# gabry1998/Self-Supervised-Anomaly-Detection

Measured on AMD Instinct MI355X. Metric: train images/sec + anomaly-maps/sec, ResNet-18 256x256 bs256, higher is better.
Workload: dtype f32; 1 GPU; ResNet-18 256x256 bs256 self-sup train + anomaly map, 1xMI355X, synthetic images (BASELINE configs[1]); images_per_gpu=256, global_batch=256, patches_per_image=841, bank_rows=588, parallelism=dp1 (256 images), train_step_launch=hipGraph segments, train_graph_segments=1

## Files before the change

### include/ssad.h

```cpp
#ifndef SSAD_H
#define SSAD_H
#include <stddef.h>
#include <stdint.h>

#ifdef __cplusplus
extern "C" {
#endif

#define SSAD_VERSION 100

int ssad_version(void);
const char* ssad_last_error(void);

int ssad_repack_oihw_to_ohwi(const float* w_oihw, float* w_ohwi, int O, int I, int KH, int KW, void* stream);
int ssad_repack_ohwi_to_oihw(const float* w_ohwi, float* w_oihw, int O, int I, int KH, int KW, void* stream);
int ssad_pack_stem_weight(const float* w_oihw, float* wk, void* stream);
int ssad_pack_stem_weight_ohwi(const float* w_ohwi, float* wk, void* stream);

int ssad_stem_fwd(const float* img, int B, int H, int W, int patch_dim, int patch_stride, int Hv, int Wv,
                  const float* wk, const float* scale, const float* shift, int relu, int hwnc, float* out, void* stream);
int ssad_stem_stats_rows(void);
int ssad_stem_fwd_stats(const float* img, int B, int H, int W, int Hv, int Wv, const float* wk, float* out, float eps,
                        float momentum, float* mean, float* invstd, float* running_mean, float* running_var, double* workspace,
                        void* stream);
// ... 11 lines not shown
int ssad_conv_igemm_fwd(const float* in, const float* w_ohwi, float* out, const float* scale, const float* shift,
                        const float* residual, int relu, int64_t N, int H, int W, int Cin, int Cout, int KH, int KW,
                        int stride, int pad, void* stream);

int ssad_conv_igemm_fwd_hwnc(const float* in, const float* w_ohwi, float* out, const float* scale, const float* shift,
                             const float* residual, int relu, int64_t N, int H, int W, int Cin, int Cout, int KH, int KW,
                             int stride, int pad, void* stream);

int ssad_conv_igemm_fwd_hwnc_ring(const float* in, const float* w_ohwi, float* out, const float* scale, const float* shift,
                                  const float* residual, int relu, int64_t N, int H, int W, int Cin, int Cout, int KH, int KW,
                                  int stride, int pad, int skip_lo, int skip_hi, void* stream);
int ssad_patch_gather_hwnc(const float* dense, float* out, int64_t B, int prow, int pcol, int shift, int Hd, int Wd, int C,
                           int H, int W, int lo, int hi, void* stream);
int ssad_patch_gather_hwnc_band(const float* dense, float* out, int64_t B, int prow, int pcol, int shift, int Hd, int Wd, int C,
                                int H, int W, int lo, int hi, int ilo, int ihi, void* stream);

int ssad_conv_igemm_tile(int64_t N, int H, int W, int Cin, int Cout, int KH, int KW, int stride, int pad, int mode);
int ssad_conv_igemm_tile_id(int64_t N, int H, int W, int Cin, int Cout, int KH, int KW, int stride, int pad, int mode);

int ssad_gap_fwd(const float* in, float* out, int64_t N, int HW, int C, int out_stride, int out_offset, int hwnc,
                 void* stream);

int ssad_l2_normalize_rows(const float* x, float* out, int64_t N, int D, void* stream);
int ssad_cosine_knn_mean(const float* sim, float* out, int64_t Nq, int Nb, int k, void* stream);

int ssad_blur_relu_bilinear(const float* maps, float* out, int n, int h, int w, int ksize, int target, void* stream);

int ssad_gradcam_map(const float* act, const float* alpha, float* out, int64_t B, int HW, int C, int alpha_stride,
                     void* stream);

// ... 292 lines not shown
```

### self-supervised-anomaly-detection_amd/csrc/conv_igemm.hip

```cpp
#include "common.h"
#include <stdlib.h>
#include <type_traits>

#ifndef IGEMM_ABL
#define IGEMM_ABL 0
#endif
#ifndef IGEMM_VAR
#define IGEMM_VAR 4
#endif
#ifndef IGEMM_EPI
#define IGEMM_EPI 1
#endif


#ifndef IGEMM_BUFLD
#define IGEMM_BUFLD 1
#endif

#ifndef IGEMM_TRACE
#define IGEMM_TRACE 0
#endif
#if IGEMM_TRACE
__device__ unsigned long long* g_ig_trace;
#define IG_STAMP(i) do { if (threadIdx.x == 0 && g_ig_trace) g_ig_trace[((size_t)blockIdx.y * gridDim.x + blockIdx.x) * 8 + (i)] = __builtin_readcyclecounter(); } while (0)
// ... 15 lines not shown
    const float* shift;
    const float* residual;
    const uint8_t* res_mask;
    int64_t M;
    int64_t N;
    int H, W, Cin, Ho, Wo, Cout, KH, KW, stride, pad, relu;
    int K;
    int hwnc;
    int cls_start[5];
    int cls_id[4];
    double* stats;
    int skip_lo, skip_hi;
    int pos_lpt;
    int pos_sg;
    int pos_chunk;
    unsigned char pos_tab[64];
};

template <int BM, int BN, int TM, int TN, int BK, int TS, bool POS, bool DB = true, int BF = 0, bool IO = false>
__global__ __launch_bounds__((BM / (32 * TM)) * (BN / (32 * TN)) * 64, (TM * TN > 8 || (TM * TN == 8 && BK >= 32)) ? 1 : 2)
void conv_igemm_f32_kernel(ConvParams p) {
    static_assert(!IO || BF == 2, "half tensors go with fp16 operands");
    using io_t = std::conditional_t<IO, hf, float>;
    constexpr int PE = IO ? 8 : 4;
    constexpr int NT = (BM / (32 * TM)) * (BN / (32 * TN)) * 64;
    constexpr int LDK = BF == 6 ? 3 * BK + 8 : (BF == 3 ? 2 * BK + 8 : (BF ? BK + 8 : BK + 4));
    constexpr int ESZ = BF ? 2 : 4;
    constexpr int CPR = BK / PE;
    constexpr int RPP = NT / CPR;
    constexpr int WN = BN / (32 * TN);
    constexpr int AR = BM / RPP;
// ... 4 lines not shown
    extern __shared__ __attribute__((aligned(16))) float lds[];

    const int tid = threadIdx.x, lane = tid & 63, wave = tid >> 6;
    const int r = lane & 31, h = lane >> 5;
    const int wm = wave / WN, wn = wave % WN;
    const int n0 = blockIdx.y * BN;
    IG_STAMP(0);
#if IGEMM_TRACE
    if (threadIdx.x == 0 && g_ig_trace)
        g_ig_trace[((size_t)blockIdx.y * gridDim.x + blockIdx.x) * 8 + 7] =
            ((unsigned long long)__builtin_amdgcn_s_getreg((31 << 11) | 20) << 32) | __builtin_amdgcn_s_getreg((31 << 11) | 4);
#endif
    const int sc = tid % CPR, sr = tid / CPR;
    const int HoWo = p.Ho * p.Wo;
    const int ntaps = p.KH * p.KW;
    const int64_t in_sp = p.hwnc ? p.N * p.Cin : (int64_t)p.Cin;
    const int64_t in_sn = p.hwnc ? (int64_t)p.Cin : (int64_t)p.H * p.W * p.Cin;
    const io_t* zero = (const io_t*)g_zero_page;
    const io_t* const tin = (const io_t*)p.in;
    const io_t* const twt = (const io_t*)p.wt;

    int64_t m0;
    int pos = 0;
    unsigned tapmask = ntaps >= 32 ? ~0u : ((1u << ntaps) - 1);
    if (POS) {
        if (p.pos_lpt == 2) {
            const unsigned x = blockIdx.x & 7, j = blockIdx.x >> 3;
            const unsigned per_blk = (unsigned)p.pos_chunk * (unsigned)HoWo;
            const unsigned blk = j / per_blk, r = j - blk * per_blk;
            const unsigned pi = r / (unsigned)p.pos_chunk, g = r - pi * (unsigned)p.pos_chunk;
            const unsigned sg = (blk * (unsigned)p.pos_chunk + g) * 8u + x;
            if (sg >= (unsigned)p.pos_sg) return;
            pos = p.pos_tab[pi];
            m0 = (int64_t)sg * BM;
        } else if (p.pos_lpt) {
            const unsigned per_chunk = (unsigned)p.pos_chunk * (unsigned)HoWo;
            const unsigned chunk = blockIdx.x / per_chunk, in_chunk = blockIdx.x - chunk * per_chunk;
            const unsigned first = chunk * (unsigned)p.pos_chunk;
            const unsigned here = min((unsigned)p.pos_chunk, (unsigned)p.pos_sg - first);
            const unsigned pi = in_chunk / here;
            if (pi >= (unsigned)HoWo) return;
            pos = p.pos_tab[pi];
            m0 = (int64_t)(first + in_chunk - pi * here) * BM;
        } else {
        const int stream = blockIdx.x & 31;
        const int64_t j = blockIdx.x >> 5;
        const int64_t q = j / HoWo;
        pos = (int)(j - q * HoWo);
        m0 = (q * 32 + stream) * BM;
        }
        if (m0 >= p.N) return;
        const int oy = pos / p.Wo, ox = pos - oy * p.Wo;
        if (oy >= p.skip_lo && oy <= p.skip_hi && ox >= p.skip_lo && ox <= p.skip_hi) return;
        tapmask = 0;
        for (int ky = 0, t = 0; ky < p.KH; ++ky)
            for (int kx = 0; kx < p.KW; ++kx, ++t) {
                const int y = oy * p.stride - p.pad + ky, x = ox * p.stride - p.pad + kx;
                if ((unsigned)y < (unsigned)p.H && (unsigned)x < (unsigned)p.W) tapmask |= 1u << t;
            }
    } else {
        m0 = (int64_t)blockIdx.x * BM;
    }
    int cpy = 0, cpx = 0, Hc = 1, Wc = 1;
// ... 24 lines not shown
            return ok;
        }
        const bool ok = m < p.M;
        const int64_t mm = ok ? m : 0;
        n = mm / HoWo;
        const int rem = (int)(mm - n * HoWo);
        oy = rem / p.Wo;
        ox = rem - oy * p.Wo;
        return ok;
    };

    constexpr bool BUFA = IGEMM_BUFLD != 0, BUFB = IGEMM_BUFLD != 0;
    constexpr unsigned OOB = 0x80000000u;
    constexpr int SRD3 = 0x00020000;
    int64_t a_org = 0;
    unsigned a_voff[AR], b_voff[BR];
    const io_t* a_ptr[AR];
    unsigned a_mask[AR];
    int a_iy[AR], a_ix[AR];
#pragma unroll
    for (int i = 0; i < AR; ++i) {
        const int64_t m = m0 + sr + RPP * i;
        int64_t n;
        int oy, ox;
        bool ok;
        if (POS) {
            ok = m < p.N;
            n = ok ? m : 0;
            oy = pos / p.Wo;
            ox = pos - oy * p.Wo;
        } else {
            ok = decode_row(m, n, oy, ox);
        }
        const int iy0 = oy * p.stride - p.pad, ix0 = ox * p.stride - p.pad;
        a_iy[i] = iy0;
        a_ix[i] = ix0;
        unsigned mk = 0;
        if (POS) {
            mk = ok ? tapmask : 0u;
        } else if (ok) {
            for (int ky = 0, t = 0; ky < p.KH; ++ky)
                for (int kx = 0; kx < p.KW; ++kx, ++t) {
                    int y = iy0 + ky, x = ix0 + kx;
                    bool v = true;
                    if (TS > 1) {
                        v = y >= 0 && x >= 0 && (y % TS) == 0 && (x % TS) == 0;
                        y /= TS;
                        x /= TS;
                    }
                    if (v && (unsigned)y < (unsigned)p.H && (unsigned)x < (unsigned)p.W) mk |= 1u << t;
                }
            mk &= tapmask;
        }
        a_mask[i] = (IGEMM_ABL & 2) ? 0u : mk;
        a_ptr[i] = TS > 1 ? tin + n * in_sn + sc * PE : tin + n * in_sn + ((int64_t)iy0 * p.W + ix0) * in_sp + sc * PE;
        if (BUFA) {
            if (POS) {
                a_org = m0 * in_sn + ((int64_t)iy0 * p.W + ix0) * in_sp;
                a_voff[i] = (ok && !(IGEMM_ABL & 2)) ? (unsigned)(((int64_t)(sr + RPP * i) * in_sn + sc * PE) * (int64_t)sizeof(io_t)) : OOB;
            } else if (TS > 1) {
                const int64_t nf = (m0 < Mc ? m0 : 0) / (Hc * Wc);
                const int mg = (p.pad + 1) / 2;
                a_org = nf * in_sn - ((int64_t)mg * p.W + mg) * in_sp;
                const int64_t R = (n - nf) * in_sn + ((int64_t)((oy - cpy) / 2 + mg) * p.W + (ox - cpx) / 2 + mg) * in_sp + sc * PE;
                a_voff[i] = ok ? (unsigned)(R * (int64_t)sizeof(io_t)) : OOB;
            } else {
                const int64_t nf = (m0 < p.M ? m0 : 0) / HoWo;
                a_org = nf * in_sn - ((int64_t)p.pad * p.W + p.pad) * in_sp;
                const int64_t R = (n - nf) * in_sn + ((int64_t)(iy0 + p.pad) * p.W + ix0 + p.pad) * in_sp + sc * PE;
                a_voff[i] = ok ? (unsigned)(R * (int64_t)sizeof(io_t)) : OOB;
            }
        }
    }
    const io_t* b_ptr[BR];
// ... 380 lines not shown
    {
        float sum = 0.f;
#pragma unroll
        for (int i = 0; i < TM; ++i)
#pragma unroll
            for (int j = 0; j < TN; ++j)
#pragma unroll
                for (int e = 0; e < 16; ++e) sum += acc[i][j][e];
        if (sum == 123.456f) p.out[0] = sum;
        return;
    }
#endif
    {
    int64_t R0 = m0, RS = 1, limit = p.M - m0;
    if (POS) {
        limit = p.N - m0;
        if (p.hwnc) { R0 = (int64_t)pos * p.N + m0; RS = 1; }
        else { R0 = m0 * HoWo + pos; RS = HoWo; }
    }
    if (IGEMM_EPI && !IO && TS == 1 && limit >= BM && n0 + BN <= p.Cout) {
        const int64_t pitch = RS * p.Cout;
        const int lrow0 = wm * 32 * TM + 4 * h;
        const int colb = n0 + wn * 32 * TN + r;
        const int64_t lane_off = (R0 + (int64_t)lrow0 * RS) * p.Cout + colb;
        float* outp = p.out + lane_off;
        float scl[TN], sft[TN];
#pragma unroll
        for (int j = 0; j < TN; ++j) {
            scl[j] = p.scale ? p.scale[colb + 32 * j] : 1.f;
            sft[j] = p.shift ? p.shift[colb + 32 * j] : 0.f;
        }
        double st0[TN], st1[TN];
// ... 141 lines not shown
                st0 += v;
                st1 += v * v;
            }
        }
        int64_t o[NPASS];
        f32x4 res[NPASS];
        f16x4 rraw[NPASS];
        unsigned mkq[NPASS];
#pragma unroll
        for (int q = 0; q < NPASS; ++q) {
            const int lr = rr + q * RP;
            int64_t row = m0 + ((lr >> 5) * TM + i) * 32 + (lr & 31);
            bool ok = col_ok;
            if (POS) {
                ok = ok && row < p.N;
                row = p.hwnc ? (int64_t)pos * p.N + row : row * HoWo + pos;
            } else if (TS > 1) {
                int64_t n;
                int oy, ox;
                ok = decode_row(row, n, oy, ox) && ok;
                row = (n * p.Ho + oy) * p.Wo + ox;
            } else {
                ok = ok && row < p.M;
            }
            o[q] = ok ? row * p.Cout + col : -1;
            if (IO) rraw[q] = *(const f16x4*)((aligned && ok && p.residual) ? (const void*)((const hf*)p.residual + o[q]) : (const void*)g_zero_page);
            else res[q] = *(const f32x4*)((aligned && ok && p.residual) ? p.residual + o[q] : g_zero_page);
            mkq[q] = 0xfu;
            if (aligned && ok && p.res_mask) mkq[q] = p.res_mask[o[q] >> 2];
        }
#pragma unroll
// ... 79 lines not shown
    constexpr int stage_bytes = (DB ? 2 : 1) * (BM + BN) *
                                (BF == 6 ? (3 * BK + 8) * 2 : (BF == 3 ? (2 * BK + 8) * 2 : (BF ? (BK + 8) * 2 : (BK + 4) * 4)));
    constexpr int epi_bytes = (BM / TM) * (BN + 4) * 4;
    constexpr int lds_min = (stage_bytes > epi_bytes ? stage_bytes : epi_bytes) + ((IGEMM_ABL & 64) ? 40 * 1024 : 0);
    static const int lds_pad = getenv(BN == 64 ? "SSAD_CONV_LDS_PAD_64" : "SSAD_CONV_LDS_PAD_128")
                                   ? atoi(getenv(BN == 64 ? "SSAD_CONV_LDS_PAD_64" : "SSAD_CONV_LDS_PAD_128")) : 0;
    const int lds_bytes = lds_min + lds_pad;
    static bool attr_set = false;
    if (!attr_set) {
        (void)hipFuncSetAttribute((const void*)conv_igemm_f32_kernel<BM, BN, TM, TN, BK, TS, POS, DB, BF, IO>,
                                  hipFuncAttributeMaxDynamicSharedMemorySize, lds_bytes);
        attr_set = true;
    }
    ConvParams q = p;
    q.pos_lpt = 0;
    if (POS) sort_positions(q, (int)cdiv64(p.N, BM));
    int64_t gx = POS ? (q.pos_lpt == 2 ? cdiv64(cdiv64(q.pos_sg, 8), q.pos_chunk) * q.pos_chunk * p.Ho * p.Wo * 8
                        : q.pos_lpt ? cdiv64(q.pos_sg, q.pos_chunk) * q.pos_chunk * p.Ho * p.Wo
                                    : cdiv64(cdiv64(p.N, BM), 32) * 32 * p.Ho * p.Wo)
                     : cdiv64(p.M, BM);
    if (TS > 1) {
        int taps[4];
        for (int c = 0; c < 4; ++c) {
            taps[c] = 0;
            for (int ky = 0; ky < p.KH; ++ky)
                for (int kx = 0; kx < p.KW; ++kx)
                    taps[c] += (((c >> 1) - p.pad + ky) & 1) == 0 && (((c & 1) - p.pad + kx) & 1) == 0;
            q.cls_id[c] = c;
        }
        for (int i = 1; i < 4; ++i)
            for (int j = i; j > 0 && taps[q.cls_id[j]] > taps[q.cls_id[j - 1]]; --j) { int t = q.cls_id[j]; q.cls_id[j] = q.cls_id[j - 1]; q.cls_id[j - 1] = t; }
        gx = 0;
        for (int c = 0; c < 4; ++c) {
            q.cls_start[c] = (int)gx;
// ... 87 lines not shown
        default: return launch<128, 128, 2, 2, 32, TS, POS>(p, st);
    }
}

enum IgemmEntry { E_FWD = 0, E_HWNC = 1, E_RING = 2, E_STATS = 3, E_DGRAD = 4 };

static bool posmajor_rows(IgemmEntry e, const ConvParams& p) {
    if (e == E_HWNC || e == E_RING) return true;
    return e == E_FWD && p.pad > 0 && p.N >= 128 && p.Ho * p.Wo <= 4;
}

static ConvParams dgrad_params(int64_t N, int Hy, int Wy, int Cout, int Hx, int Wx, int Cin, int KH, int KW, int pad) {
    ConvParams p;
    p.pos_lpt = 0; p.pos_sg = 0; p.pos_chunk = 1;
    p.skip_lo = 1; p.skip_hi = 0;
    p.in = nullptr; p.wt = nullptr; p.out = nullptr; p.scale = nullptr; p.shift = nullptr; p.residual = nullptr; p.res_mask = nullptr;
    p.H = Hy; p.W = Wy; p.Cin = Cout; p.Cout = Cin; p.KH = KH; p.KW = KW; p.relu = 0;
    p.stride = 1; p.pad = KH - 1 - pad; p.N = N; p.hwnc = 0;
    p.Ho = Hx; p.Wo = Wx; p.stats = nullptr;
    p.M = N * Hx * Wx;
    p.K = KH * KW * Cout;
    return p;
}

static bool tile_span_ok(const ConvParams& p, bool posmajor, int elt_bytes, int ts = 1) {
    const int64_t image = (int64_t)p.H * p.W * p.Cin * elt_bytes;
    if (posmajor) return p.hwnc || 256 * image < ((int64_t)1 << 31);
    const int64_t rows_per_image = ts > 1 ? (int64_t)(p.Ho / 2) * (p.Wo / 2) : (int64_t)p.Ho * p.Wo;
    return (256 / (rows_per_image > 0 ? rows_per_image : 1) + 2) * image < ((int64_t)1 << 31);
}

int conv_fwd_impl(const float* in, const float* w_ohwi, float* out, const float* scale, const float* shift,
                  const float* residual, int relu, int64_t N, int H, int W, int Cin, int Cout, int KH, int KW, int stride,
                  int pad, int hwnc, void* stream, int bf16 = 0, double* stats = nullptr, int* stat_rows = nullptr, int io16 = 0,
                  int skip_lo = 1, int skip_hi = 0) {
    SSAD_CHECK_ARG(in && w_ohwi && out, "null pointer");
    SSAD_CHECK_ARG(!io16 || (bf16 == 2 && !hwnc && Cout % 4 == 0), "half tensors: fp16 operands, NHWC, Cout % 4 == 0");
    SSAD_CHECK_ARG(N > 0 && H > 0 && W > 0 && Cin > 0 && Cout > 0, "empty shape");
    if ((bf16 == 0 || bf16 == 1 || bf16 == 2) && !io16 && !hwnc && KH == 1 && KW == 1 && H == 1 && W == 1 && stride == 1 && pad == 0 &&
        ssad_linear_small_ok(in, w_ohwi, N, Cin))
        return ssad_linear_small_launch(in, w_ohwi, out, scale, shift, residual, relu, (int)N, Cin, Cout, stats, stat_rows, stream, bf16);
    SSAD_CHECK_ARG(Cin % KALIGN == 0, "Cin must be a multiple of 32");
    SSAD_CHECK_ARG(KH > 0 && KW > 0 && stride > 0 && pad >= 0 && KH * KW <= 32, "bad filter geometry (<= 32 taps)");
    ConvParams p;
    p.pos_lpt = 0; p.pos_sg = 0; p.pos_chunk = 1;
    p.skip_lo = skip_lo; p.skip_hi = skip_hi;
    SSAD_CHECK_ARG(skip_lo > skip_hi || hwnc, "a skipped rectangle of output positions: position-major tensors only");
    p.in = in; p.wt = w_ohwi; p.out = out; p.scale = scale; p.shift = shift; p.residual = residual; p.res_mask = nullptr;
    p.H = H; p.W = W; p.Cin = Cin; p.Cout = Cout; p.KH = KH; p.KW = KW; p.stride = stride; p.pad = pad; p.relu = relu;
    p.Ho = (H + 2 * pad - KH) / stride + 1;
    p.Wo = (W + 2 * pad - KW) / stride + 1;
    SSAD_CHECK_ARG(p.Ho > 0 && p.Wo > 0, "empty output");
    p.M = N * p.Ho * p.Wo;
    p.N = N;
    p.K = KH * KW * Cin;
    p.hwnc = hwnc;
    p.stats = stats;
    const bool posmajor = posmajor_rows(hwnc ? (skip_lo <= skip_hi ? E_RING : E_HWNC) : stats ? E_STATS : E_FWD, p);
    SSAD_CHECK_ARG(cdiv64(p.M, 128) + 32 * p.Ho * p.Wo < (int64_t)2147483647, "M too large for one launch");
    SSAD_CHECK_ARG(tile_span_ok(p, posmajor, io16 ? 2 : 4), "input images too large: the rows of a tile must span less than 2 GB");
    hipStream_t st = (hipStream_t)stream;
    int rows;
    SSAD_CHECK_ARG(bf16 == 0 || bf16 == 1 || bf16 == 2 || bf16 == 3 || bf16 == 6,
                   "operand mode: 0 (fp32), 1 (bf16), 2 (fp16), 3 (bf16x3), 6 (bf16x6)");
    if (bf16 == 6) {
        rows = posmajor ? dispatch_x6<1, true>(p, st) : dispatch_x6<1, false>(p, st);
    } else if (bf16 == 3) {
        rows = posmajor ? dispatch_x3<1, true>(p, st) : dispatch_x3<1, false>(p, st);
    } else if (bf16) {
// ... 59 lines not shown
extern "C" int ssad_conv_igemm_fwd_hwnc(const float* in, const float* w_ohwi, float* out, const float* scale,
                                        const float* shift, const float* residual, int relu, int64_t N, int H, int W,
                                        int Cin, int Cout, int KH, int KW, int stride, int pad, void* stream) {
    return conv_fwd_impl(in, w_ohwi, out, scale, shift, residual, relu, N, H, W, Cin, Cout, KH, KW, stride, pad, 1, stream);
}

extern "C" int ssad_conv_igemm_fwd_hwnc_ring(const float* in, const float* w_ohwi, float* out, const float* scale,
                                             const float* shift, const float* residual, int relu, int64_t N, int H, int W,
                                             int Cin, int Cout, int KH, int KW, int stride, int pad, int skip_lo, int skip_hi,
                                             void* stream) {
    SSAD_CHECK_ARG(skip_lo >= 0 && skip_hi < H && skip_hi < W, "skipped square outside the map");
    return conv_fwd_impl(in, w_ohwi, out, scale, shift, residual, relu, N, H, W, Cin, Cout, KH, KW, stride, pad, 1, stream, 0, nullptr,
                         nullptr, 0, skip_lo, skip_hi);
}

extern "C" int ssad_conv_igemm_tile_id(int64_t N, int H, int W, int Cin, int Cout, int KH, int KW, int stride, int pad, int mode) {
    const int Ho = (H + 2 * pad - KH) / stride + 1, Wo = (W + 2 * pad - KW) / stride + 1;
    ConvParams p;
    if (mode == E_DGRAD) {
        p = dgrad_params(N, Ho, Wo, Cout, H, W, Cin, KH, KW, pad);
    } else {
        p.N = N; p.H = H; p.W = W; p.Cin = Cin; p.Cout = Cout; p.KH = KH; p.KW = KW; p.stride = stride; p.pad = pad;
        p.skip_lo = mode == E_RING ? 0 : 1; p.skip_hi = 0;
        p.Ho = Ho; p.Wo = Wo;
        p.M = N * p.Ho * p.Wo;
    }
    if (posmajor_rows((IgemmEntry)mode, p)) return 100 + (int)pick_tile<true>(p);
    const IgemmTile t = pick_tile<false>(p);
    return t == T_256x256 ? T_128x128 : (int)t;
}

extern "C" int ssad_conv_igemm_tile(int64_t N, int H, int W, int Cin, int Cout, int KH, int KW, int stride, int pad, int mode) {
    static const int dims[13][3] = {{256, 64, 16}, {256, 64, 32}, {128, 64, 32}, {256, 128, 32}, {256, 128, 32}, {128, 256, 32},
                                    {64, 64, 32}, {128, 128, 32}, {256, 256, 32}, {128, 64, 32}, {128, 64, 16}, {128, 128, 16}, {128, 256, 16}};
    const int id = ssad_conv_igemm_tile_id(N, H, W, Cin, Cout, KH, KW, stride, pad, mode), t = id % 100;
    const int code = dims[t][0] * 100000 + dims[t][1] * 100 + dims[t][2];
    return id >= 100 ? -code : code;
}
// ... 103 lines not shown
```

### self-supervised-anomaly-detection_amd/csrc/misc.hip

```cpp
#include "common.h"
#include <stdarg.h>

static thread_local char g_err[512] = "";

void ssad_set_error(const char* fmt, ...) {
    va_list ap;
    va_start(ap, fmt);
    vsnprintf(g_err, sizeof(g_err), fmt, ap);
    va_end(ap);
}

extern "C" const char* ssad_last_error(void) { return g_err; }
extern "C" int ssad_version(void) { return 100; }

namespace {

__global__ void repack_kernel(const float* __restrict__ src, float* __restrict__ dst, int O, int I, int KH, int KW,
                              int to_ohwi) {
    int64_t idx = (int64_t)blockIdx.x * blockDim.x + threadIdx.x;
    int64_t total = (int64_t)O * I * KH * KW;
    if (idx >= total) return;
    int ci = (int)(idx % I);
    int64_t t = idx / I;
    int kx = (int)(t % KW); t /= KW;
// ... 305 lines not shown
    const int64_t N = B * prow * pcol;
    const int side = hi - lo + 1;
    const int iside = ilo > ihi ? 0 : ihi - ilo + 1;
    SSAD_CHECK_ARG(cdiv64(N * (C / 4), 256) < (int64_t)2147483647 && side * side <= 65535, "too large for one launch");
    hipLaunchKernelGGL(patch_gather_hwnc_kernel, dim3((unsigned)cdiv64(N * (C / 4), 256), side * side - iside * iside), dim3(256), 0,
                       (hipStream_t)stream, (const f32x4*)dense, (f32x4*)out, N, prow, pcol, shift, Hd, Wd, C / 4, W, lo, side, ilo, iside);
    SSAD_CHECK_LAUNCH();
    return 0;
}

extern "C" int ssad_patch_gather_hwnc(const float* dense, float* out, int64_t B, int prow, int pcol, int shift, int Hd, int Wd, int C,
                                      int H, int W, int lo, int hi, void* stream) {
    return ssad_patch_gather_hwnc_band(dense, out, B, prow, pcol, shift, Hd, Wd, C, H, W, lo, hi, 1, 0, stream);
}

extern "C" int ssad_gradcam_map(const float* act, const float* alpha, float* out, int64_t B, int HW, int C, int alpha_stride,
                                void* stream) {
    SSAD_CHECK_ARG(act && alpha && out && B > 0 && HW > 0 && C > 0 && alpha_stride >= C, "bad argument");
    const int64_t rows = B * HW;
    hipLaunchKernelGGL(gradcam_map_kernel, dim3((unsigned)cdiv64(rows, 4)), dim3(256), 0, (hipStream_t)stream, act, alpha, out,
                       rows, HW, C, alpha_stride);
    SSAD_CHECK_LAUNCH();
    return 0;
}

extern "C" int ssad_l2_normalize_rows(const float* x, float* out, int64_t N, int D, void* stream) {
    SSAD_CHECK_ARG(x && out && N > 0 && D > 0, "bad argument");
    hipLaunchKernelGGL(l2norm_rows_kernel, dim3((unsigned)cdiv64(N, 4)), dim3(256), 0, (hipStream_t)stream, x, out, N, D);
    SSAD_CHECK_LAUNCH();
    return 0;
// ... 33 lines not shown
```

### self-supervised-anomaly-detection_amd/self_supervised/_hip.py

```python
import ctypes
import os

import torch

_HERE = os.path.dirname(os.path.abspath(__file__))
LIB_PATH = os.path.join(os.path.dirname(_HERE), "lib", "libssad_hip.so")

_c_fp = ctypes.c_void_p
_c_i = ctypes.c_int
_c_l = ctypes.c_int64
_c_f = ctypes.c_float

SIGNATURES = {
    "ssad_repack_oihw_to_ohwi": [_c_fp, _c_fp, _c_i, _c_i, _c_i, _c_i, _c_fp],
    "ssad_repack_ohwi_to_oihw": [_c_fp, _c_fp, _c_i, _c_i, _c_i, _c_i, _c_fp],
    "ssad_pack_stem_weight": [_c_fp, _c_fp, _c_fp],
    "ssad_pack_stem_weight_ohwi": [_c_fp, _c_fp, _c_fp],
    "ssad_pack_stem_weight16_ohwi": [_c_fp, _c_fp, _c_i, _c_fp],
    "ssad_stem_fwd": [_c_fp, _c_i, _c_i, _c_i, _c_i, _c_i, _c_i, _c_i, _c_fp, _c_fp, _c_fp, _c_i, _c_i, _c_fp, _c_fp],
    "ssad_stem_stats_rows": [],
    "ssad_stem_fwd_stats": [_c_fp, _c_i, _c_i, _c_i, _c_i, _c_i, _c_fp, _c_fp, _c_f, _c_f, _c_fp, _c_fp, _c_fp, _c_fp, _c_fp, _c_fp],
    "ssad_pack_stem_weight_folded": [_c_fp, _c_fp, _c_fp],
    "ssad_stem_patch_pool_fwd": [_c_fp, _c_i, _c_i, _c_i, _c_i, _c_fp, _c_fp, _c_fp, _c_i, _c_fp, _c_fp],
    "ssad_stem_patch_pool_fwd_ring": [_c_fp, _c_i, _c_i, _c_i, _c_i, _c_fp, _c_fp, _c_fp, _c_i, _c_i, _c_i, _c_fp, _c_fp],
    "ssad_stem_patch_border_fwd": [_c_fp, _c_i, _c_i, _c_i, _c_i, _c_fp, _c_fp, _c_fp, _c_fp, _c_fp],
    "ssad_maxpool3x3s2_fwd": [_c_fp, _c_fp, _c_l, _c_i, _c_i, _c_i, _c_i, _c_fp],
    "ssad_conv_igemm_fwd": [_c_fp, _c_fp, _c_fp, _c_fp, _c_fp, _c_fp, _c_i, _c_l, _c_i, _c_i, _c_i, _c_i, _c_i, _c_i,
                            _c_i, _c_i, _c_fp],
    "ssad_conv_igemm_fwd_hwnc": [_c_fp, _c_fp, _c_fp, _c_fp, _c_fp, _c_fp, _c_i, _c_l, _c_i, _c_i, _c_i, _c_i, _c_i, _c_i,
                                 _c_i, _c_i, _c_fp],
    "ssad_conv_igemm_fwd_hwnc_ring": [_c_fp, _c_fp, _c_fp, _c_fp, _c_fp, _c_fp, _c_i, _c_l, _c_i, _c_i, _c_i, _c_i, _c_i, _c_i,
                                      _c_i, _c_i, _c_i, _c_i, _c_fp],
    "ssad_patch_gather_hwnc": [_c_fp, _c_fp, _c_l, _c_i, _c_i, _c_i, _c_i, _c_i, _c_i, _c_i, _c_i, _c_i, _c_i, _c_fp],
    "ssad_patch_gather_hwnc_band": [_c_fp, _c_fp, _c_l, _c_i, _c_i, _c_i, _c_i, _c_i, _c_i, _c_i, _c_i, _c_i, _c_i, _c_i, _c_i, _c_fp],
    "ssad_conv_igemm_tile": [_c_l, _c_i, _c_i, _c_i, _c_i, _c_i, _c_i, _c_i, _c_i, _c_i],
    "ssad_conv_igemm_tile_id": [_c_l, _c_i, _c_i, _c_i, _c_i, _c_i, _c_i, _c_i, _c_i, _c_i],
    "ssad_gap_fwd": [_c_fp, _c_fp, _c_l, _c_i, _c_i, _c_i, _c_i, _c_i, _c_fp],
    "ssad_l2_normalize_rows": [_c_fp, _c_fp, _c_l, _c_i, _c_fp],
    "ssad_cosine_knn_mean": [_c_fp, _c_fp, _c_l, _c_i, _c_i, _c_fp],
    "ssad_cosine_knn_fused": [_c_fp, _c_fp, _c_fp, _c_l, _c_i, _c_i, _c_i, _c_fp],
    "ssad_cosine_knn_split": [_c_fp, _c_fp, _c_fp, _c_fp, _c_l, _c_i, _c_i, _c_i, _c_i, _c_fp],
    "ssad_coreset_greedy": [_c_fp, _c_l, _c_i, _c_i, _c_l, _c_i, _c_fp, _c_fp, _c_fp, _c_fp, _c_fp, _c_fp],
    "ssad_gaussian_fit_stats": [_c_fp, _c_l, _c_i, _c_i, _c_fp, _c_fp, _c_fp, _c_fp],
    "ssad_mahalanobis_fused": [_c_fp, _c_fp, _c_fp, _c_fp, _c_fp, _c_l, _c_i, _c_i, _c_fp],
    "ssad_blur_relu_bilinear": [_c_fp, _c_fp, _c_i, _c_i, _c_i, _c_i, _c_i, _c_fp],
    "ssad_flip_transpose_weight": [_c_fp, _c_fp, _c_i, _c_i, _c_i, _c_i, _c_fp],
    "ssad_flip_transpose_batch": [_c_fp, _c_fp, ctypes.POINTER(ctypes.c_int64), _c_i, _c_fp],
    "ssad_conv_igemm_dgrad": [_c_fp, _c_fp, _c_fp, _c_fp, _c_l, _c_i, _c_i, _c_i, _c_i, _c_i, _c_i, _c_i, _c_i, _c_i, _c_i,
                              _c_fp],
# ... 206 lines not shown
```

### self-supervised-anomaly-detection_amd/self_supervised/engine.py

```python
import torch
from torch import nn

import os as _os

from . import ops

BLOCKS = [("layer1", 64, 64, 1), ("layer2", 64, 128, 2), ("layer3", 128, 256, 2), ("layer4", 256, 512, 2)]


def math_mode():
    m = _os.environ.get("SSAD_MATH", "f32").lower()
    return 6 if m in ("bf16x6", "x6") else 3 if m in ("bf16x3", "x3") else 0


class _Block(nn.Module):

    def __init__(self, cin, cout, stride):
        super().__init__()
        self.conv1 = nn.Conv2d(cin, cout, 3, stride, 1, bias=False)
        self.bn1 = nn.BatchNorm2d(cout)
        self.conv2 = nn.Conv2d(cout, cout, 3, 1, 1, bias=False)
        self.bn2 = nn.BatchNorm2d(cout)
        self.downsample = None
        if stride != 1 or cin != cout:
# ... 116 lines not shown
    return pooled


def _trunk_eval_dedup(plan, x, patch_stride, layer_outputs, pooled, conv):
    b, _, h, w = x.shape
    prow, pcol = (h - 32) // patch_stride + 1, (w - 32) // patch_stride + 1
    shift = patch_stride // 2
    band = _os.environ.get("SSAD_GATHER_BAND", "1") != "0"
    dn = ops.stem_fwd(x, plan.stem_w, plan.stem_s, plan.stem_t, True, resize_to=(2 * h, 2 * w))
    dn = ops.maxpool3x3s2_fwd(dn)
    if band and _os.environ.get("SSAD_STEM_BORDER", "1") != "0":
        a = ops.stem_patch_border_fwd(x, plan.stem_wf, plan.stem_s, plan.stem_t, patch_stride)
        ops.patch_gather_hwnc(dn, a, prow, pcol, shift, 2, 14, 4, 12)
    else:
        a = ops.stem_patch_pool_fwd(x, plan.stem_wf, plan.stem_s, plan.stem_t, patch_stride, True, (4, 12) if band else None)
    offs, off = {}, 0
    for k in ("layer1", "layer2", "layer3"):
        if k in layer_outputs:
            offs[k] = off
            off += {"layer1": 64, "layer2": 128, "layer3": 256}[k]
    offs["layer4"] = off
    for i, (name, d) in enumerate(plan.blocks):
        s = d["stride"]
        if name == "layer1":
            lo, hi = 3 + 2 * i, 13 - 2 * i
            dt = ops.conv3x3_c64_eval(dn, d["w1"], d["s1"], d["t1"], None, True)
            dn2 = ops.conv3x3_c64_eval(dt, d["w2"], d["s2"], d["t2"], dn, True)
            t = ops.conv_fwd_hwnc_ring(a, d["w1"], d["s1"], d["t1"], None, True, lo, hi)
            ops.patch_gather_hwnc(dt, t, prow, pcol, shift, lo, hi, *((lo + 2, hi - 2) if band else (1, 0)))
            a2 = ops.conv_fwd_hwnc_ring(t, d["w2"], d["s2"], d["t2"], a, True, lo + 1, hi - 1)
            ops.patch_gather_hwnc(dn2, a2, prow, pcol, shift, lo + 1, hi - 1, *((lo + 3, hi - 3) if band and i == 0 else (1, 0)))
            a, dn = a2, dn2
        else:
            idt = a
            if "wd" in d:
                idt = conv(a, d["wd"], d["sd"], d["td"], None, False, s, 0)
            t = conv(a, d["w1"], d["s1"], d["t1"], None, True, s, 1)
            a = conv(t, d["w2"], d["s2"], d["t2"], idt, True, 1, 1)
        if i % 2 == 1 and name in offs:
            ops.gap_fwd(a, pooled, offs[name], True)
    return pooled


def head_eval(plan, pooled):
    f = pooled
# ... 6 lines not shown
```

### self-supervised-anomaly-detection_amd/self_supervised/ops.py

```python
import os

import torch

from . import _hip


PROFILE = None


def _new(shape, like):
    return torch.empty(shape, device=like.device, dtype=torch.float32)


def _newh(shape, like):
    return torch.empty(shape, device=like.device, dtype=torch.float16)


def _is_h(t):
    return t is not None and t.dtype == torch.float16


def _p(t, allow_none=False):
    return _hip.ptr(t, allow_none, torch.float16 if _is_h(t) else torch.float32)

# ... 257 lines not shown

def conv_fwd_hwnc_ring(x, w_ohwi, scale, shift, residual, relu, skip_lo, skip_hi):
    h, w, n, cin = x.shape
    cout, kh, kw, cin2 = w_ohwi.shape
    assert cin == cin2 and (kh, kw) == (3, 3) and 0 <= skip_lo <= skip_hi < min(h, w)
    out = _new((h, w, n, cout), x)
    side = skip_hi - skip_lo + 1
    ring = h * w - side * side
    taps = _inbounds_taps(h, w, 3, 3, 1, 1) - 9 * side * side if PROFILE is not None else 0
    _run("conv_igemm_pos_f32", 2.0 * n * ring * cout * 9 * cin, 4.0 * (x.numel() + n * ring * cout * (2 if residual is not None else 1) + w_ohwi.numel()),
         lambda: _hip.lib().ssad_conv_igemm_fwd_hwnc_ring(_hip.ptr(x), _hip.ptr(w_ohwi), _hip.ptr(out), _hip.ptr(scale, True),
                                                          _hip.ptr(shift, True), _hip.ptr(residual, True), int(relu), n, h, w,
                                                          cin, cout, 3, 3, 1, 1, skip_lo, skip_hi, _hip.stream()),
         exec_flops=2.0 * n * cout * cin * taps if PROFILE is not None else None,
         tile=lambda: igemm_tile_name(n, h, w, cin, cout, 3, 3, 1, 1, IGEMM_RING))
    return out


def patch_gather_hwnc(dense, out, prow, pcol, shift, lo, hi, ilo=1, ihi=0):
    b, hd, wd, c = dense.shape
    h, w, n, c2 = out.shape
    assert c == c2 and n == b * prow * pcol
    side, iside = hi - lo + 1, max(ihi - ilo + 1, 0)
    _run("patch_gather", 0.0, 8.0 * n * (side * side - iside * iside) * c,
         lambda: _hip.lib().ssad_patch_gather_hwnc_band(_hip.ptr(dense), _hip.ptr(out), b, prow, pcol, shift, hd, wd, c, h, w, lo, hi,
                                                        ilo, ihi, _hip.stream()))
    return out


def conv_fwd(x, w_ohwi, scale=None, shift=None, residual=None, relu=False, stride=1, pad=0, bf16=False):
# ... 895 lines not shown
```

Measured before the change: 8191 images/sec.

## Share overlapping ring-strip conv outputs between neighbouring patches instead of recomputing

In the patch-wise anomaly-map path, overlapping patches (stride smaller than the computed window) recompute identical ring conv outputs. The ring conv is split into strip launches that compute only the non-overlapping windows and edge rows of patches, using a listed position table and a row remapping. A new copy kernel then fills the shared strip positions from neighbouring patches. This cuts redundant FLOPs in layer1 ring convs, at the cost of more launches, extra copy traffic and complex index maps.

```diff
diff --git a/include/ssad.h b/include/ssad.h
--- a/include/ssad.h
+++ b/include/ssad.h
@@ -49,6 +49,13 @@
                            int H, int W, int lo, int hi, void* stream);
 int ssad_patch_gather_hwnc_band(const float* dense, float* out, int64_t B, int prow, int pcol, int shift, int Hd, int Wd, int C,
                                 int H, int W, int lo, int hi, int ilo, int ihi, void* stream);
+
+int ssad_conv_igemm_fwd_hwnc_strip(const float* in, const float* w_ohwi, float* out, const float* scale, const float* shift,
+                                   const float* residual, int relu, int64_t N, int H, int W, int Cin, int Cout, int KH, int KW,
+                                   int stride, int pad, int skip_lo, int skip_hi, int corners, int tb_lo, int tb_hi, int lr_lo,
+                                   int lr_hi, int row_P, int row_S, int row_O, int64_t rows, void* stream);
+int ssad_patch_strip_copy_hwnc(float* out, int64_t B, int prow, int pcol, int shift, int C, int H, int W, int lo, int hi,
+                               void* stream);
 
 int ssad_conv_igemm_tile(int64_t N, int H, int W, int Cin, int Cout, int KH, int KW, int stride, int pad, int mode);
 int ssad_conv_igemm_tile_id(int64_t N, int H, int W, int Cin, int Cout, int KH, int KW, int stride, int pad, int mode);
diff --git a/self-supervised-anomaly-detection_amd/csrc/conv_igemm.hip b/self-supervised-anomaly-detection_amd/csrc/conv_igemm.hip
--- a/self-supervised-anomaly-detection_amd/csrc/conv_igemm.hip
+++ b/self-supervised-anomaly-detection_amd/csrc/conv_igemm.hip
@@ -53,7 +53,10 @@
     int pos_lpt;
     int pos_sg;
     int pos_chunk;
-    unsigned char pos_tab[64];
+    int pos_cnt;
+    int row_P, row_S, row_O;
+    int64_t Nt;
+    unsigned char pos_tab[256];
 };
 
 template <int BM, int BN, int TM, int TN, int BK, int TS, bool POS, bool DB = true, int BF = 0, bool IO = false>
@@ -88,7 +91,7 @@
     const int sc = tid % CPR, sr = tid / CPR;
     const int HoWo = p.Ho * p.Wo;
     const int ntaps = p.KH * p.KW;
-    const int64_t in_sp = p.hwnc ? p.N * p.Cin : (int64_t)p.Cin;
+    const int64_t in_sp = p.hwnc ? p.Nt * p.Cin : (int64_t)p.Cin;
     const int64_t in_sn = p.hwnc ? (int64_t)p.Cin : (int64_t)p.H * p.W * p.Cin;
     const io_t* zero = (const io_t*)g_zero_page;
     const io_t* const tin = (const io_t*)p.in;
@@ -119,8 +122,10 @@
         } else {
         const int stream = blockIdx.x & 31;
         const int64_t j = blockIdx.x >> 5;
-        const int64_t q = j / HoWo;
-        pos = (int)(j - q * HoWo);
+        const int npos = p.pos_cnt ? p.pos_cnt : HoWo;
+        const int64_t q = j / npos;
+        pos = (int)(j - q * npos);
+        if (p.pos_cnt) pos = p.pos_tab[pos];
         m0 = (q * 32 + stream) * BM;
         }
         if (m0 >= p.N) return;
@@ -175,6 +180,12 @@
     constexpr unsigned OOB = 0x80000000u;
     constexpr int SRD3 = 0x00020000;
     int64_t a_org = 0;
+    auto row_sample = [&](int64_t m) -> int64_t {
+        if (!POS || !p.row_P) return m;
+        const int64_t g = m / p.row_P;
+        return g * p.row_S + p.row_O + (m - g * p.row_P);
+    };
+    const int64_t ns0 = POS ? row_sample(m0) : 0;
     unsigned a_voff[AR], b_voff[BR];
     const io_t* a_ptr[AR];
     unsigned a_mask[AR];
@@ -187,7 +198,7 @@
         bool ok;
         if (POS) {
             ok = m < p.N;
-            n = ok ? m : 0;
+            n = ok ? row_sample(m) : ns0;
             oy = pos / p.Wo;
             ox = pos - oy * p.Wo;
         } else {
@@ -217,8 +228,8 @@
         a_ptr[i] = TS > 1 ? tin + n * in_sn + sc * PE : tin + n * in_sn + ((int64_t)iy0 * p.W + ix0) * in_sp + sc * PE;
         if (BUFA) {
             if (POS) {
-                a_org = m0 * in_sn + ((int64_t)iy0 * p.W + ix0) * in_sp;
-                a_voff[i] = (ok && !(IGEMM_ABL & 2)) ? (unsigned)(((int64_t)(sr + RPP * i) * in_sn + sc * PE) * (int64_t)sizeof(io_t)) : OOB;
+                a_org = ns0 * in_sn + ((int64_t)iy0 * p.W + ix0) * in_sp;
+                a_voff[i] = (ok && !(IGEMM_ABL & 2)) ? (unsigned)(((n - ns0) * in_sn + sc * PE) * (int64_t)sizeof(io_t)) : OOB;
             } else if (TS > 1) {
                 const int64_t nf = (m0 < Mc ? m0 : 0) / (Hc * Wc);
                 const int mg = (p.pad + 1) / 2;
@@ -629,8 +640,8 @@
     {
     int64_t R0 = m0, RS = 1, limit = p.M - m0;
     if (POS) {
-        limit = p.N - m0;
-        if (p.hwnc) { R0 = (int64_t)pos * p.N + m0; RS = 1; }
+        limit = p.row_P ? 0 : p.N - m0;
+        if (p.hwnc) { R0 = (int64_t)pos * p.Nt + m0; RS = 1; }
         else { R0 = m0 * HoWo + pos; RS = HoWo; }
     }
     if (IGEMM_EPI && !IO && TS == 1 && limit >= BM && n0 + BN <= p.Cout) {
@@ -802,7 +813,7 @@
             bool ok = col_ok;
             if (POS) {
                 ok = ok && row < p.N;
-                row = p.hwnc ? (int64_t)pos * p.N + row : row * HoWo + pos;
+                row = p.hwnc ? (int64_t)pos * p.Nt + (ok ? row_sample(row) : 0) : row * HoWo + pos;
             } else if (TS > 1) {
                 int64_t n;
                 int oy, ox;
@@ -912,10 +923,10 @@
     }
     ConvParams q = p;
     q.pos_lpt = 0;
-    if (POS) sort_positions(q, (int)cdiv64(p.N, BM));
+    if (POS && !p.pos_cnt) sort_positions(q, (int)cdiv64(p.N, BM));
     int64_t gx = POS ? (q.pos_lpt == 2 ? cdiv64(cdiv64(q.pos_sg, 8), q.pos_chunk) * q.pos_chunk * p.Ho * p.Wo * 8
                         : q.pos_lpt ? cdiv64(q.pos_sg, q.pos_chunk) * q.pos_chunk * p.Ho * p.Wo
-                                    : cdiv64(cdiv64(p.N, BM), 32) * 32 * p.Ho * p.Wo)
+                                    : cdiv64(cdiv64(p.N, BM), 32) * 32 * (p.pos_cnt ? p.pos_cnt : p.Ho * p.Wo))
                      : cdiv64(p.M, BM);
     if (TS > 1) {
         int taps[4];
@@ -1033,6 +1044,7 @@
     ConvParams p;
     p.pos_lpt = 0; p.pos_sg = 0; p.pos_chunk = 1;
     p.skip_lo = 1; p.skip_hi = 0;
+    p.pos_cnt = 0; p.row_P = 0; p.row_S = 0; p.row_O = 0; p.Nt = N;
     p.in = nullptr; p.wt = nullptr; p.out = nullptr; p.scale = nullptr; p.shift = nullptr; p.residual = nullptr; p.res_mask = nullptr;
     p.H = Hy; p.W = Wy; p.Cin = Cout; p.Cout = Cin; p.KH = KH; p.KW = KW; p.relu = 0;
     p.stride = 1; p.pad = KH - 1 - pad; p.N = N; p.hwnc = 0;
@@ -1049,10 +1061,17 @@
     return (256 / (rows_per_image > 0 ? rows_per_image : 1) + 2) * image < ((int64_t)1 << 31);
 }
 
+struct StripSet {
+    int pos_cnt;
+    unsigned char pos[256];
+    int row_P, row_S, row_O;
+    int64_t rows;
+};
+
 int conv_fwd_impl(const float* in, const float* w_ohwi, float* out, const float* scale, const float* shift,
                   const float* residual, int relu, int64_t N, int H, int W, int Cin, int Cout, int KH, int KW, int stride,
                   int pad, int hwnc, void* stream, int bf16 = 0, double* stats = nullptr, int* stat_rows = nullptr, int io16 = 0,
-                  int skip_lo = 1, int skip_hi = 0) {
+                  int skip_lo = 1, int skip_hi = 0, const StripSet* strip = nullptr) {
     SSAD_CHECK_ARG(in && w_ohwi && out, "null pointer");
     SSAD_CHECK_ARG(!io16 || (bf16 == 2 && !hwnc && Cout % 4 == 0), "half tensors: fp16 operands, NHWC, Cout % 4 == 0");
     SSAD_CHECK_ARG(N > 0 && H > 0 && W > 0 && Cin > 0 && Cout > 0, "empty shape");
@@ -1072,6 +1091,23 @@
     SSAD_CHECK_ARG(p.Ho > 0 && p.Wo > 0, "empty output");
     p.M = N * p.Ho * p.Wo;
     p.N = N;
+    p.Nt = N;
+    p.pos_cnt = 0; p.row_P = 0; p.row_S = 0; p.row_O = 0;
+    if (strip) {
+        SSAD_CHECK_ARG(hwnc && bf16 == 0 && !stats && skip_lo <= skip_hi && p.Ho * p.Wo <= 256 && strip->pos_cnt > 0,
+                       "a listed position set: exact-fp32 ring launches over position-major maps of <= 256 positions");
+        p.pos_cnt = strip->pos_cnt;
+        for (int i = 0; i < strip->pos_cnt; ++i) p.pos_tab[i] = strip->pos[i];
+        if (strip->row_P) {
+            const int64_t last = (strip->rows - 1) / strip->row_P * strip->row_S + strip->row_O + (strip->rows - 1) % strip->row_P;
+            SSAD_CHECK_ARG(strip->rows > 0 && strip->row_P > 0 && strip->row_S >= strip->row_P && strip->row_O >= 0 && last < N,
+                           "row map outside the tensors");
+            SSAD_CHECK_ARG((256 / strip->row_P + 2) * (int64_t)strip->row_S * Cin * 4 < ((int64_t)1 << 31), "row map: a tile spans 2 GB");
+            p.row_P = strip->row_P; p.row_S = strip->row_S; p.row_O = strip->row_O;
+            p.N = strip->rows;
+            p.M = p.N * p.Ho * p.Wo;
+        }
+    }
     p.K = KH * KW * Cin;
     p.hwnc = hwnc;
     p.stats = stats;
@@ -1161,6 +1197,29 @@
                          nullptr, 0, skip_lo, skip_hi);
 }
 
+extern "C" int ssad_conv_igemm_fwd_hwnc_strip(const float* in, const float* w_ohwi, float* out, const float* scale,
+                                              const float* shift, const float* residual, int relu, int64_t N, int H, int W,
+                                              int Cin, int Cout, int KH, int KW, int stride, int pad, int skip_lo, int skip_hi,
+                                              int corners, int tb_lo, int tb_hi, int lr_lo, int lr_hi, int row_P, int row_S,
+                                              int row_O, int64_t rows, void* stream) {
+    SSAD_CHECK_ARG(H > 0 && W > 0 && KH > 0 && KW > 0 && stride > 0 && pad >= 0, "bad geometry");
+    const int Ho = (H + 2 * pad - KH) / stride + 1, Wo = (W + 2 * pad - KW) / stride + 1;
+    SSAD_CHECK_ARG(skip_lo >= 0 && skip_lo <= skip_hi && skip_hi < Ho && skip_hi < Wo, "skipped square outside the map");
+    SSAD_CHECK_ARG(Ho > 0 && Wo > 0 && Ho * Wo <= 256, "a listed position set: maps of <= 256 positions");
+    StripSet s;
+    s.pos_cnt = 0;
+    for (int oy = 0; oy < Ho; ++oy)
+        for (int ox = 0; ox < Wo; ++ox) {
+            const bool iy = oy >= skip_lo && oy <= skip_hi, ix = ox >= skip_lo && ox <= skip_hi;
+            const bool take = (!iy && !ix) ? corners != 0 : (!iy && ix) ? (ox >= tb_lo && ox <= tb_hi) : (iy && !ix) ? (oy >= lr_lo && oy <= lr_hi) : false;
+            if (take) s.pos[s.pos_cnt++] = (unsigned char)(oy * Wo + ox);
+        }
+    SSAD_CHECK_ARG(s.pos_cnt > 0, "empty position set");
+    s.row_P = row_P; s.row_S = row_S; s.row_O = row_O; s.rows = rows;
+    return conv_fwd_impl(in, w_ohwi, out, scale, shift, residual, relu, N, H, W, Cin, Cout, KH, KW, stride, pad, 1, stream, 0, nullptr,
+                         nullptr, 0, skip_lo, skip_hi, &s);
+}
+
 extern "C" int ssad_conv_igemm_tile_id(int64_t N, int H, int W, int Cin, int Cout, int KH, int KW, int stride, int pad, int mode) {
     const int Ho = (H + 2 * pad - KH) / stride + 1, Wo = (W + 2 * pad - KW) / stride + 1;
     ConvParams p;
@@ -1169,6 +1228,7 @@
     } else {
         p.N = N; p.H = H; p.W = W; p.Cin = Cin; p.Cout = Cout; p.KH = KH; p.KW = KW; p.stride = stride; p.pad = pad;
         p.skip_lo = mode == E_RING ? 0 : 1; p.skip_hi = 0;
+        p.pos_cnt = 0; p.row_P = 0; p.row_S = 0; p.row_O = 0; p.Nt = N;
         p.Ho = Ho; p.Wo = Wo;
         p.M = N * p.Ho * p.Wo;
     }
diff --git a/self-supervised-anomaly-detection_amd/csrc/misc.hip b/self-supervised-anomaly-detection_amd/csrc/misc.hip
--- a/self-supervised-anomaly-detection_amd/csrc/misc.hip
+++ b/self-supervised-anomaly-detection_amd/csrc/misc.hip
@@ -343,6 +343,53 @@
     return ssad_patch_gather_hwnc_band(dense, out, B, prow, pcol, shift, Hd, Wd, C, H, W, lo, hi, 1, 0, stream);
 }
 
+namespace {
+__global__ __launch_bounds__(256) void patch_strip_copy_hwnc_kernel(f32x4* out, int64_t N, int prow, int pcol, int shift, int C4, int H,
+                                                                   int W, int lo, int side) {
+    const int64_t i = (int64_t)blockIdx.x * 256 + threadIdx.x;
+    if (i >= N * C4) return;
+    const int c4 = (int)(i % C4);
+    const int64_t n = i / C4;
+    const int rem = (int)(n % ((int64_t)prow * pcol));
+    const int pr = rem / pcol, pc = rem - pr * pcol;
+    const int wrem = side - shift, tb = (H - side) * wrem;
+    int u, v, k;
+    int64_t src_n;
+    if ((int)blockIdx.y < tb) {
+        const int a = (int)blockIdx.y / wrem;
+        u = a < lo ? a : a + side;
+        v = lo + shift + (int)blockIdx.y % wrem;
+        k = (v - lo) / shift;
+        if (pc + k >= pcol) return;
+        src_n = n + k;
+        out[(((int64_t)u * W + v) * N + n) * C4 + c4] = out[(((int64_t)u * W + v - shift * k) * N + src_n) * C4 + c4];
+    } else {
+        const int kk = (int)blockIdx.y - tb, ws = W - side, b = kk % ws;
+        v = b < lo ? b : b + side;
+        u = lo + shift + kk / ws;
+        k = (u - lo) / shift;
+        if (pr + k >= prow) return;
+        src_n = n + (int64_t)k * pcol;
+        out[(((int64_t)u * W + v) * N + n) * C4 + c4] = out[(((int64_t)(u - shift * k) * W + v) * N + src_n) * C4 + c4];
+    }
+}
+}
+
+extern "C" int ssad_patch_strip_copy_hwnc(float* out, int64_t B, int prow, int pcol, int shift, int C, int H, int W, int lo, int hi,
+                                          void* stream) {
+    SSAD_CHECK_ARG(out && B > 0 && prow > 0 && pcol > 0 && shift > 0 && C > 0 && C % 4 == 0, "bad argument");
+    SSAD_CHECK_ARG(lo >= 0 && hi >= lo && hi < H && hi < W, "the square must lie inside the map");
+    const int side = hi - lo + 1;
+    SSAD_CHECK_ARG(shift < side && (H > side || W > side), "nothing to copy: the computed windows cover the strips");
+    const int64_t N = B * prow * pcol;
+    const int npos = (H - side) * (side - shift) + (side - shift) * (W - side);
+    SSAD_CHECK_ARG(cdiv64(N * (C / 4), 256) < (int64_t)2147483647 && npos <= 65535, "too large for one launch");
+    hipLaunchKernelGGL(patch_strip_copy_hwnc_kernel, dim3((unsigned)cdiv64(N * (C / 4), 256), npos), dim3(256), 0, (hipStream_t)stream,
+                       (f32x4*)out, N, prow, pcol, shift, C / 4, H, W, lo, side);
+    SSAD_CHECK_LAUNCH();
+    return 0;
+}
+
 extern "C" int ssad_gradcam_map(const float* act, const float* alpha, float* out, int64_t B, int HW, int C, int alpha_stride,
                                 void* stream) {
     SSAD_CHECK_ARG(act && alpha && out && B > 0 && HW > 0 && C > 0 && alpha_stride >= C, "bad argument");
diff --git a/self-supervised-anomaly-detection_amd/self_supervised/_hip.py b/self-supervised-anomaly-detection_amd/self_supervised/_hip.py
--- a/self-supervised-anomaly-detection_amd/self_supervised/_hip.py
+++ b/self-supervised-anomaly-detection_amd/self_supervised/_hip.py
@@ -33,6 +33,9 @@
                                       _c_i, _c_i, _c_i, _c_i, _c_fp],
     "ssad_patch_gather_hwnc": [_c_fp, _c_fp, _c_l, _c_i, _c_i, _c_i, _c_i, _c_i, _c_i, _c_i, _c_i, _c_i, _c_i, _c_fp],
     "ssad_patch_gather_hwnc_band": [_c_fp, _c_fp, _c_l, _c_i, _c_i, _c_i, _c_i, _c_i, _c_i, _c_i, _c_i, _c_i, _c_i, _c_i, _c_i, _c_fp],
+    "ssad_conv_igemm_fwd_hwnc_strip": [_c_fp, _c_fp, _c_fp, _c_fp, _c_fp, _c_fp, _c_i, _c_l, _c_i, _c_i, _c_i, _c_i, _c_i, _c_i,
+                                       _c_i, _c_i, _c_i, _c_i, _c_i, _c_i, _c_i, _c_i, _c_i, _c_i, _c_i, _c_i, _c_l, _c_fp],
+    "ssad_patch_strip_copy_hwnc": [_c_fp, _c_l, _c_i, _c_i, _c_i, _c_i, _c_i, _c_i, _c_i, _c_i, _c_fp],
     "ssad_conv_igemm_tile": [_c_l, _c_i, _c_i, _c_i, _c_i, _c_i, _c_i, _c_i, _c_i, _c_i],
     "ssad_conv_igemm_tile_id": [_c_l, _c_i, _c_i, _c_i, _c_i, _c_i, _c_i, _c_i, _c_i, _c_i],
     "ssad_gap_fwd": [_c_fp, _c_fp, _c_l, _c_i, _c_i, _c_i, _c_i, _c_i, _c_fp],
diff --git a/self-supervised-anomaly-detection_amd/self_supervised/engine.py b/self-supervised-anomaly-detection_amd/self_supervised/engine.py
--- a/self-supervised-anomaly-detection_amd/self_supervised/engine.py
+++ b/self-supervised-anomaly-detection_amd/self_supervised/engine.py
@@ -154,6 +154,24 @@
         ops.patch_gather_hwnc(dn, a, prow, pcol, shift, 2, 14, 4, 12)
     else:
         a = ops.stem_patch_pool_fwd(x, plan.stem_wf, plan.stem_s, plan.stem_t, patch_stride, True, (4, 12) if band else None)
+    strips = _os.environ.get("SSAD_STRIP_SHARE", "1") != "0"
+
+    def ring(x_, w_, s_, t_, res, lo, hi):
+        side = hi - lo + 1
+        e = -(-(side - shift) // shift)
+        if not strips or shift >= side or prow <= e or pcol <= e:
+            return ops.conv_fwd_hwnc_ring(x_, w_, s_, t_, res, True, lo, hi)
+        hh, ww, n, _ = x_.shape
+        out = torch.empty((hh, ww, n, w_.shape[0]), device=x_.device, dtype=torch.float32)
+        win, none = (lo, lo + shift - 1), (1, 0)
+        ops.conv_fwd_hwnc_strip(x_, w_, s_, t_, res, True, lo, hi, True, win, win, out)
+        for k in range(1, e + 1):
+            rest = (lo + k * shift, hi)
+            ops.conv_fwd_hwnc_strip(x_, w_, s_, t_, res, True, lo, hi, False, rest, none, out, (1, pcol, pcol - k, b * prow))
+            ops.conv_fwd_hwnc_strip(x_, w_, s_, t_, res, True, lo, hi, False, none, rest, out,
+                                    (pcol, prow * pcol, (prow - k) * pcol, b * pcol))
+        return ops.patch_strip_copy_hwnc(out, prow, pcol, shift, lo, hi)
+
     offs, off = {}, 0
     for k in ("layer1", "layer2", "layer3"):
         if k in layer_outputs:
@@ -166,9 +184,9 @@
             lo, hi = 3 + 2 * i, 13 - 2 * i
             dt = ops.conv3x3_c64_eval(dn, d["w1"], d["s1"], d["t1"], None, True)
             dn2 = ops.conv3x3_c64_eval(dt, d["w2"], d["s2"], d["t2"], dn, True)
-            t = ops.conv_fwd_hwnc_ring(a, d["w1"], d["s1"], d["t1"], None, True, lo, hi)
+            t = ring(a, d["w1"], d["s1"], d["t1"], None, lo, hi)
             ops.patch_gather_hwnc(dt, t, prow, pcol, shift, lo, hi, *((lo + 2, hi - 2) if band else (1, 0)))
-            a2 = ops.conv_fwd_hwnc_ring(t, d["w2"], d["s2"], d["t2"], a, True, lo + 1, hi - 1)
+            a2 = ring(t, d["w2"], d["s2"], d["t2"], a, lo + 1, hi - 1)
             ops.patch_gather_hwnc(dn2, a2, prow, pcol, shift, lo + 1, hi - 1, *((lo + 3, hi - 3) if band and i == 0 else (1, 0)))
             a, dn = a2, dn2
         else:
diff --git a/self-supervised-anomaly-detection_amd/self_supervised/ops.py b/self-supervised-anomaly-detection_amd/self_supervised/ops.py
--- a/self-supervised-anomaly-detection_amd/self_supervised/ops.py
+++ b/self-supervised-anomaly-detection_amd/self_supervised/ops.py
@@ -295,6 +295,46 @@
                                                           cin, cout, 3, 3, 1, 1, skip_lo, skip_hi, _hip.stream()),
          exec_flops=2.0 * n * cout * cin * taps if PROFILE is not None else None,
          tile=lambda: igemm_tile_name(n, h, w, cin, cout, 3, 3, 1, 1, IGEMM_RING))
+    return out
+
+
+def strip_positions(h, w, skip_lo, skip_hi, corners, tb, lr):
+    oy, ox = torch.arange(h).view(h, 1), torch.arange(w).view(1, w)
+    iy, ix = (oy >= skip_lo) & (oy <= skip_hi), (ox >= skip_lo) & (ox <= skip_hi)
+    m = ~iy & ix & (ox >= tb[0]) & (ox <= tb[1]) | iy & ~ix & (oy >= lr[0]) & (oy <= lr[1])
+    return m | (~iy & ~ix) if corners else m
+
+
+def conv_fwd_hwnc_strip(x, w_ohwi, scale, shift, residual, relu, skip_lo, skip_hi, corners, tb, lr, out, rowmap=None):
+    h, w, n, cin = x.shape
+    cout, kh, kw, cin2 = w_ohwi.shape
+    assert cin == cin2 and (kh, kw) == (3, 3) and out.shape == (h, w, n, cout)
+    p, s, o, rows = rowmap if rowmap is not None else (0, 0, 0, n)
+    npos = taps = 0
+    if PROFILE is not None:
+        m = strip_positions(h, w, skip_lo, skip_hi, corners, tb, lr)
+        ty = torch.tensor([sum(1 for k in range(3) if 0 <= y - 1 + k < h) for y in range(h)]).view(h, 1)
+        tx = torch.tensor([sum(1 for k in range(3) if 0 <= x_ - 1 + k < w) for x_ in range(w)]).view(1, w)
+        npos, taps = int(m.sum()), int((ty * tx)[m].sum())
+    _run("conv_igemm_pos_f32", 2.0 * rows * npos * cout * 9 * cin,
+         4.0 * (rows * npos * (cin + cout * (2 if residual is not None else 1)) + w_ohwi.numel()),
+         lambda: _hip.lib().ssad_conv_igemm_fwd_hwnc_strip(_hip.ptr(x), _hip.ptr(w_ohwi), _hip.ptr(out), _hip.ptr(scale, True),
+                                                           _hip.ptr(shift, True), _hip.ptr(residual, True), int(relu), n, h, w,
+                                                           cin, cout, 3, 3, 1, 1, skip_lo, skip_hi, int(corners), tb[0], tb[1],
+                                                           lr[0], lr[1], p, s, o, rows, _hip.stream()),
+         exec_flops=2.0 * rows * cout * cin * taps if PROFILE is not None else None,
+         tile=lambda: igemm_tile_name(rows, h, w, cin, cout, 3, 3, 1, 1, IGEMM_RING))
+    return out
+
+
+def patch_strip_copy_hwnc(out, prow, pcol, shift, lo, hi):
+    h, w, n, c = out.shape
+    b = n // (prow * pcol)
+    assert n == b * prow * pcol
+    side = hi - lo + 1
+    npos = (h - side + w - side) * (side - shift)
+    _run("patch_strip_copy", 0.0, 8.0 * n * npos * c,
+         lambda: _hip.lib().ssad_patch_strip_copy_hwnc(_hip.ptr(out), b, prow, pcol, shift, c, h, w, lo, hi, _hip.stream()))
     return out
 
 
```

New measurement: 8178 images/sec. About the same (-0.2%).
